# aras-p/UnityGaussianSplatting

Hardware: AMD Instinct MI355X
Metric: Msplats/s rendered (sort+view+composite+resolve), bicycle-sized synthetic 6,131,954 splats, 1200x797, Medium; ms/frame in ms_per_step (higher is better)
Workload: dtype f32; 1 GPU; bicycle-sized synthetic 6,131,954 splats, 1200x797, Medium; sort_mode=visible_in_flight, frames_in_flight=2, frames_in_flight_impl=library, splats=6131954, views=1, views_per_rank=1, blend=exact, sort_nth_frame=1, tile_pairs_P=4376060, tile=32x16, visible_splats=1563698, parallelism=single GPU, rccl_ranks=0

## Files before the change

unitygaussiansplatting_amd/csrc/gs_device_math.h:

```cpp
#pragma once
#include <stdint.h>

#if defined(__HIPCC__)
#include <hip/hip_runtime.h>
#include <hip/hip_fp16.h>
#define GS_HD __host__ __device__ __forceinline__
#else
#include <cmath>
#include <cstring>
#define GS_HD inline
#endif

#ifndef GS_CULL_EXTENT
#define GS_CULL_EXTENT 2.8285f
#endif

namespace gsm {

struct AssetView {
    const uint8_t* pos;
    const uint8_t* other;
    const uint8_t* color;
    const uint8_t* sh;
    const uint8_t* chunk;
// ... 678 lines not shown
    const float lambda2 = fmaxf(mid - radius, 0.1f);
    float dvx = cov01, dvy = lambda1 - cov00;
    const float invLen = 1.0f / sqrtf(dot2f(dvx, dvy, dvx, dvy));
    dvx *= invLen; dvy *= invLen;
    dvy = -dvy;
    const float s1 = fminf(sqrtf(2.0f * lambda1), 4096.0f), s2 = fminf(sqrtf(2.0f * lambda2), 4096.0f);
    view.axis1[0] = s1 * dvx; view.axis1[1] = s1 * dvy;
    view.axis2[0] = s2 * dvy; view.axis2[1] = s2 * (-dvx);

    const float al = fminf(col.w * P.opacityScale, 65000.0f);
    view.color[1] = f32tof16(al);
}

template <class SHSource>
GS_HD void CalcViewColor(const AssetView& a, const FrameConsts& P, uint32_t idx, ViewPartial& vp, SHSource& shsrc) {
    ViewData& view = vp.view;
    const V4 col = vp.col;
    const V3 shMin = vp.shMin, shMax = vp.shMax;
    const bool shLerp = vp.shLerp;
    const float wx = vp.wx, wy = vp.wy, wz = vp.wz;
    const float dwx = P.camx - wx, dwy = P.camy - wy, dwz = P.camz - wz;
    float ox = mrow3(P.w2o, 0, dwx, dwy, dwz), oy = mrow3(P.w2o, 1, dwx, dwy, dwz), oz = mrow3(P.w2o, 2, dwx, dwy, dwz);
    const float invN = 1.0f / sqrtf(dot3f(ox, oy, oz, ox, oy, oz));
    ox *= invN; oy *= invN; oz *= invN;
    const float dx = -ox, dy = -oy, dz = -oz;

    const bool onlySH = P.shOnly != 0;
    F2 rg = onlySH ? F2{ 0.5f, 0.5f } : F2{ col.x, col.y };
    float b = onlySH ? 0.5f : col.z;
    if (P.shOrder >= 1) {
        uint32_t shIndex = idx;
        if (a.shFmt > 3) shIndex = LoadUShort(a.other, vp.otherEnd - 2);
        shsrc.begin(a.sh + (uint64_t)shIndex * shStrideOf(a.shFmt), a.shFmt);
        const F2 minRG = { shMin.x, shMin.y }, dRG = F2{ shMax.x, shMax.y } - minRG;
        const float minB = shMin.z, dB = shMax.z - shMin.z;
        auto SHK = [&](int k) -> RGB {
            RGB s = shsrc.load_rgb(k);
            if (shLerp) { s.rg = fma2(s.rg, dRG, minRG); s.b = fmaf(s.b, dB, minB); }
            return s;
        };
        auto MUL = [](float w, const RGB& s) -> RGB { return { F2{ w, w } * s.rg, w * s.b }; };
        auto FMA = [](float w, const RGB& s, const RGB& acc) -> RGB { return { fma2(F2{ w, w }, s.rg, acc.rg), fmaf(w, s.b, acc.b) }; };
        {
            const RGB s1v = SHK(1), s2v = SHK(2), s3v = SHK(3);
            RGB t = MUL(dy, RGB{ -s1v.rg, -s1v.b });
            t = FMA(dz, s2v, t);
            t = FMA(dx, RGB{ -s3v.rg, -s3v.b }, t);
            rg = fma2(F2{ GS_SH_C1, GS_SH_C1 }, t.rg, rg); b = fmaf(GS_SH_C1, t.b, b);
        }
        if (P.shOrder >= 2) {
            const float xx = dx * dx, yy = dy * dy, zz = dz * dz;
            const float xy = dx * dy, yz = dy * dz, xz = dx * dz;
            {
                const float b4 = 1.0925484f * xy, b5 = -1.0925484f * yz, b6 = 0.3153916f * (fmaf(2.0f, zz, -xx) - yy),
                            b7 = -1.0925484f * xz, b8 = 0.5462742f * (xx - yy);
                RGB acc = MUL(b4, SHK(4));
                acc = FMA(b5, SHK(5), acc);
                acc = FMA(b6, SHK(6), acc);
                acc = FMA(b7, SHK(7), acc);
                acc = FMA(b8, SHK(8), acc);
                rg += acc.rg; b += acc.b;
            }
            if (P.shOrder >= 3) {
                const float b9 = (-0.5900436f * dy) * fmaf(3.0f, xx, -yy);
                const float b10 = (2.8906114f * xy) * dz;
                const float b11 = (-0.4570458f * dy) * (fmaf(4.0f, zz, -xx) - yy);
                const float b12 = (0.3731763f * dz) * (fmaf(2.0f, zz, -3.0f * xx) - 3.0f * yy);
                const float b13 = (-0.4570458f * dx) * (fmaf(4.0f, zz, -xx) - yy);
                const float b14 = (1.4453057f * dz) * (xx - yy);
                const float b15 = (-0.5900436f * dx) * fmaf(-3.0f, yy, xx);
                RGB acc = MUL(b9, SHK(9));
                acc = FMA(b10, SHK(10), acc);
                acc = FMA(b11, SHK(11), acc);
                acc = FMA(b12, SHK(12), acc);
                acc = FMA(b13, SHK(13), acc);
                acc = FMA(b14, SHK(14), acc);
                acc = FMA(b15, SHK(15), acc);
                rg += acc.rg; b += acc.b;
            }
        }
    }
    float r = rg.x, g = rg.y;
    r = fmaxf(r, 0.0f); g = fmaxf(g, 0.0f); b = fmaxf(b, 0.0f);
    view.color[0] = (f32tof16(r) << 16) | f32tof16(g);
    view.color[1] = (f32tof16(b) << 16) | (view.color[1] & 0xffffu);
}

template <class SHSource>
GS_HD ViewData CalcViewDataT(const AssetView& a, const FrameConsts& P, const EditView& E, uint32_t idx, SHSource& shsrc) {
    ViewPartial vp;
    CalcViewGeom(a, P, E, idx, vp);
    if (vp.front) CalcViewColor(a, P, idx, vp, shsrc);
    return vp.view;
}

GS_HD ViewData CalcViewData(const AssetView& a, const FrameConsts& P, const EditView& E, uint32_t idx) {
    SHFromBlob src;
    return CalcViewDataT(a, P, E, idx, src);
}

GS_HD void PixRange(float c, float e, float size, int& lo, int& hi) {
    float flo = ceilf((c - e) - 0.5f), fhi = floorf((c + e) - 0.5f);
    flo = fmaxf(flo, 0.0f); fhi = fminf(fhi, size - 1.0f);
    if (!(flo <= fhi)) { lo = 1; hi = 0; return; }
    lo = (int)flo; hi = (int)fhi;
}

constexpr uint32_t kAlphaThresholdBits = 0x3B808081u;
constexpr uint32_t kAlphaWindow = 16u;
constexpr uint32_t kAlphaWindowLo = kAlphaThresholdBits - kAlphaWindow / 2u;
GS_HD float Exp2Det(float y) {
    const float n = rintf(y);
    const float f = y - n;
    float p = 1.525273380405984e-05f;
    p = fmaf(p, f, 1.5403530393381608e-04f);
    p = fmaf(p, f, 1.3333558146428443e-03f);
    p = fmaf(p, f, 9.618129107628477e-03f);
    p = fmaf(p, f, 5.550410866482158e-02f);
    p = fmaf(p, f, 2.402265069591007e-01f);
    p = fmaf(p, f, 6.931471805599453e-01f);
    p = fmaf(p, f, 1.0f);
    return ldexpf(p, (int)n);
}
GS_HD float DecideAlpha(float alphaNative, float y, float a, bool& live) {
    const uint32_t u = f2u(alphaNative) - kAlphaWindowLo;
    if (u < kAlphaWindow) {
        const float ad = fminf(fmaxf(Exp2Det(y) * a, 0.0f), 1.0f);
        live = ad >= u2f(kAlphaThresholdBits);
        return ad;
    }
    live = (int32_t)u >= (int32_t)kAlphaWindow;
    return alphaNative;
}

GS_HD float LogDet(float x) {
    const uint32_t u = f2u(x);
    float e = (float)((int)(u >> 23) - 127);
    float m = u2f((u & 0x7fffffu) | 0x3f800000u);
    if (m > 1.41421356f) { m *= 0.5f; e += 1.0f; }
    const float t = (m - 1.0f) / (m + 1.0f);
    const float t2 = t * t;
    const float p = fmaf(t2, fmaf(t2, fmaf(t2, 1.0f / 7.0f, 0.2f), 1.0f / 3.0f), 1.0f);
    return fmaf(e, 0.69314718f, (2.0f * t) * p);
}

GS_HD bool BlockMayTouch(float bcx, float bcy, float half, float cx, float cy, float u1x, float u1y, float u2x, float u2y, float r2) {
    const float dx = bcx - cx, dy = bcy - cy;
    const float d1 = fabsf(fmaf(dy, u1y, dx * u1x)) - half * (fabsf(u1x) + fabsf(u1y));
    const float d2 = fabsf(fmaf(dy, u2y, dx * u2x)) - half * (fabsf(u2x) + fabsf(u2y));
    const float m1 = fmaxf(d1, 0.0f), m2 = fmaxf(d2, 0.0f);
    return (m1 <= 2.001f) && (m2 <= 2.001f) && (fmaf(m2, m2, m1 * m1) <= r2);
}

struct SplatFootprint {
    float cx, cy;
    int x0, x1, y0, y1;
};
GS_HD void PackPixelRect(const SplatFootprint& fp, uint32_t& rx, uint32_t& ry) {
    rx = (uint32_t)fp.x0 | ((uint32_t)fp.y0 << 16);
    ry = (uint32_t)(fp.x1 + 1) | ((uint32_t)(fp.y1 + 1) << 16);
}

GS_HD bool PrepareSplat(const ViewData& v, float W, float H, float nearClip, float farClip, SplatFootprint& fp) {
    fp.x0 = 1; fp.x1 = 0; fp.y0 = 1; fp.y1 = 0; fp.cx = 0.0f; fp.cy = 0.0f;
    const float w = v.pos[3];
    const float a = f16tof32(v.color[1]);
    const int drawable = (int)(w > 0.0f) & (int)(w >= nearClip) & (int)(w <= farClip) & (int)finite32(v.axis1[0]) & (int)finite32(v.axis1[1]) &
                         (int)finite32(v.axis2[0]) & (int)finite32(v.axis2[1]) & (int)(a >= 1.0f / 255.0f);
    if (!drawable) return false;
    const float invw = 1.0f / w;
    const float cx = fmaf(0.5f * (v.pos[0] * invw), W, 0.5f * W);
    const float cy = fmaf(-0.5f * (v.pos[1] * invw), H, 0.5f * H);
    const float a1x = v.axis1[0], a1y = v.axis1[1], a2x = v.axis2[0], a2y = v.axis2[1];
    const float d1 = dot2f(a1x, a1y, a1x, a1y), d2 = dot2f(a2x, a2y, a2x, a2y);
    const int inv1ok = (int)((f2u(d1) - 0x00200001u) <= (0x7f800000u - 0x00200001u)), inv2ok = (int)((f2u(d2) - 0x00200001u) <= (0x7f800000u - 0x00200001u));
    fp.cx = cx; fp.cy = cy;
    if (!((int)finite32(cx) & (int)finite32(cy) & inv1ok & inv2ok)) return false;
    const float exr = 2.0f * (fabsf(a1x) + fabsf(a2x)), eyr = 2.0f * (fabsf(a1y) + fabsf(a2y));
    const float slack = 0.01f;
    int x0, x1, y0, y1;
    PixRange(fp.cx, exr + slack, W, x0, x1);
    PixRange(fp.cy, eyr + slack, H, y0, y1);
    if (x0 > x1 || y0 > y1) return false;
    const float r2 = fmaf(LogDet(255.0f * a), 1.0001f, 1.0e-3f);
    const float rr = sqrtf(fmaxf(r2, 0.0f));
    const float exe = rr * sqrtf(dot2f(a1x, a2x, a1x, a2x)), eye = rr * sqrtf(dot2f(a1y, a2y, a1y, a2y));
    PixRange(fp.cx, fminf(exr, exe) + slack, W, x0, x1);
    PixRange(fp.cy, fminf(eyr, eye) + slack, H, y0, y1);
    if (x0 > x1 || y0 > y1) return true;
    fp.x0 = x0; fp.x1 = x1; fp.y0 = y0; fp.y1 = y1;
    return true;
}

}
```

unitygaussiansplatting_amd/csrc/gs_raster.hip:

```cpp
#include "gs_common.h"
#include <cstdlib>

namespace gs {

namespace {

struct RasterConsts {
    float W, H, nearClip, farClip;
    uint32_t tilesX, tilesY, width, height;
};

constexpr unsigned long long BFLAG_AGG = 1ull << 62, BFLAG_INCL = 2ull << 62, BVAL_MASK = (1ull << 62) - 1ull;
constexpr uint32_t BIN_SPIN_LIMIT = 1u << 24;

__device__ __forceinline__ float rl(float x, int b) { return __int_as_float(__builtin_amdgcn_readlane(__float_as_int(x), b)); }

__device__ __forceinline__ uint32_t wave_incl_scan_u32(uint32_t v) {
#define GS_DPP(x, ctrl, rowmask) (uint32_t)__builtin_amdgcn_update_dpp(0, (int)(x), ctrl, rowmask, 0xf, false)
    v += GS_DPP(v, 0x111, 0xf);
    v += GS_DPP(v, 0x112, 0xf);
    v += GS_DPP(v, 0x114, 0xf);
    v += GS_DPP(v, 0x118, 0xf);
    v += GS_DPP(v, 0x142, 0xa);
    v += GS_DPP(v, 0x143, 0xc);
// ... 571 lines not shown
            const uint32_t o = slot - s_off[e];
            const uint32_t twh = s_twh[e], tx0 = s_tx[e];
            uint32_t ty, tx;
            slot_to_xy(o, max(twh & 0xffffu, 1u), ty, tx);
            tiles[k] = __umul24((tx0 >> 16) + ty, tilesX) + (tx0 & 0xffffu) + tx;
            sids[k] = s_sid[e];
            live[k] = slot < s1;
        }
        if (live[SPT - 1]) {
            static_assert(SPT == 4, "four slots per thread");
            *(uint4*)(pairKeys + s0 + tid * SPT) = make_uint4(tiles[0], tiles[1], tiles[2], tiles[3]);
            *(uint4*)(pairVals + s0 + tid * SPT) = make_uint4(sids[0], sids[1], sids[2], sids[3]);
        } else {
#pragma unroll
            for (int k = 0; k < SPT; ++k) if (live[k]) { pairKeys[s0 + tid * SPT + k] = tiles[k]; pairVals[s0 + tid * SPT + k] = sids[k]; }
        }
#pragma unroll
        for (int k = 0; k < SPT; ++k) {
            if (live[k]) {
                if (TILECNT) atomicAdd(&s_tile[tiles[k]], 1u);
                else atomicAdd(&s_hist[tiles[k] & digitMask], 1u);
            }
            if (!TILECNT && PASSES >= 2) hist_add_aggregated(s_hist + 256, (tiles[k] >> digitBits) & digitMask, live[k]);
            if (!TILECNT && PASSES >= 3) hist_add_aggregated(s_hist + 512, (tiles[k] >> (2u * digitBits)) & digitMask, live[k]);
        }
    }
    __syncthreads();
    if (TILECNT) {
        for (uint32_t t = tid; t < kBinTileCounters; t += kEmitThreads) {
            const uint32_t c = s_tile[t];
            if (c) {
                atomicAdd(&s_hist[t & digitMask], c);
                if (PASSES >= 2) atomicAdd(&s_hist[256 + ((t >> digitBits) & digitMask)], c);
            }
        }
        __syncthreads();
    }
    uint32_t* myHist = pairHist + (bid % histCopies) * (uint32_t)kHistStride;
    for (int j = tid; j < PASSES * 256; j += kEmitThreads) {
        const uint32_t c = s_hist[j];
        if (c) atomicAdd(&myHist[j], c);
    }
}

__global__ __launch_bounds__(256) void tile_ranges_kernel(const uint32_t* __restrict__ pairKeys, const uint32_t* nPtr,
                                                          uint32_t* __restrict__ tileStart, uint32_t* __restrict__ tileEnd, uint32_t numTiles) {
    GS_CHAIN_PRIORITY();
    const uint32_t n = *nPtr;
    const uint32_t octs = (n + 7u) >> 3;
    for (uint32_t q = blockIdx.x * 256u + threadIdx.x; q < octs; q += gridDim.x * 256u) {
        const uint32_t j0 = q << 3;
        const uint4 ka = ((const uint4*)pairKeys)[2u * q], kb = ((const uint4*)pairKeys)[2u * q + 1u];
        const uint32_t k[10] = { j0 ? pairKeys[j0 - 1u] : 0xffffffffu, ka.x, ka.y, ka.z, ka.w, kb.x, kb.y, kb.z, kb.w,
                                 (j0 + 8u < n) ? pairKeys[j0 + 8u] : 0xffffffffu };
#pragma unroll
        for (int c = 0; c < 8; ++c) {
            const uint32_t j = j0 + (uint32_t)c;
            if (j >= n) break;
            const uint32_t t = k[c + 1];
            if (t >= numTiles) continue;
            if (j == 0 || k[c] != t) tileStart[t] = j;
            if (j == n - 1 || k[c + 2] != t) tileEnd[t] = j + 1;
        }
    }
}

__device__ __forceinline__ float mix_mul_lo(uint32_t h, float x) {
    float d;
    asm("v_fma_mix_f32 %0, %1, %2, 0 op_sel_hi:[1,0,0]" : "=v"(d) : "v"(h), "v"(x));
    return d;
}
__device__ __forceinline__ float mix_mul_hi(uint32_t h, float x) {
    float d;
    asm("v_fma_mix_f32 %0, %1, %2, 0 op_sel:[1,0,0] op_sel_hi:[1,0,0]" : "=v"(d) : "v"(h), "v"(x));
    return d;
}
__device__ __forceinline__ float mix_mul_lo_sat_after_trans(uint32_t h, float x) {
    float d;
    asm("s_nop 0\n\tv_fma_mix_f32 %0, %1, %2, 0 op_sel_hi:[1,0,0] clamp" : "=v"(d) : "v"(h), "v"(x));
    return d;
}
__device__ __forceinline__ float mix_one_minus_hi(uint32_t h) {
    float d;
    asm("v_fma_mix_f32 %0, %1, -1.0, 1.0 op_sel:[1,0,0] op_sel_hi:[1,0,0]" : "=v"(d) : "v"(h));
    return d;
}
__device__ __forceinline__ void mix_blend4(uint32_t& rg, uint32_t& ba, float pr, float pg, float pb, float pa, float t) {
    asm("v_fma_mixlo_f16 %0, %2, %6, %0 op_sel_hi:[0,0,1]\n\t"
        "v_fma_mixlo_f16 %1, %4, %6, %1 op_sel_hi:[0,0,1]\n\t"
        "v_fma_mixhi_f16 %0, %3, %6, %0 op_sel:[0,0,1] op_sel_hi:[0,0,1]\n\t"
        "v_fma_mixhi_f16 %1, %5, %6, %1 op_sel:[0,0,1] op_sel_hi:[0,0,1]"
        : "+v"(rg), "+v"(ba) : "v"(pr), "v"(pg), "v"(pb), "v"(pa), "v"(t));
}

__device__ __forceinline__ float half_lo(uint32_t u) { return (float)__builtin_bit_cast(_Float16, (unsigned short)(u & 0xffffu)); }
__device__ __forceinline__ float half_hi(uint32_t u) { return (float)__builtin_bit_cast(_Float16, (unsigned short)(u >> 16)); }
template <int MODE> struct PixelAcc;
template <> struct PixelAcc<0> {
    uint32_t rg, ba;
    __device__ __forceinline__ void load(uint2 d) { rg = d.x; ba = d.y; }
    __device__ __forceinline__ void blend(uint32_t c0, uint32_t c1, float alpha) {
        const float t = mix_one_minus_hi(ba);
        mix_blend4(rg, ba, mix_mul_hi(c0, alpha), mix_mul_lo(c0, alpha), mix_mul_hi(c1, alpha), alpha, t);
    }
    __device__ __forceinline__ void blend_src(float pr, float pg, float pb, float pa) { const float t = mix_one_minus_hi(ba); mix_blend4(rg, ba, pr, pg, pb, pa, t); }
    __device__ __forceinline__ bool finished() const { return (ba >> 16) == 0x3c00u; }
    __device__ __forceinline__ bool saturated() const { return false; }
    __device__ __forceinline__ uint2 pack() const { return make_uint2(rg, ba); }
};
template <> struct PixelAcc<1> {
    float r, g, b, a;
    __device__ __forceinline__ void load(uint2 d) {
        r = gsm::f16tof32(d.x); g = gsm::f16tof32(d.x >> 16); b = gsm::f16tof32(d.y); a = gsm::f16tof32(d.y >> 16);
    }
    __device__ __forceinline__ void blend(uint32_t c0, uint32_t c1, float alpha) {
        const float t = 1.0f - a;
        r = fmaf(mix_mul_hi(c0, alpha), t, r); g = fmaf(mix_mul_lo(c0, alpha), t, g); b = fmaf(mix_mul_hi(c1, alpha), t, b);
        a = fmaf(alpha, t, a);
    }
    __device__ __forceinline__ void blend_src(float pr, float pg, float pb, float pa) { const float t = 1.0f - a; r = fmaf(pr, t, r); g = fmaf(pg, t, g); b = fmaf(pb, t, b); a = fmaf(pa, t, a); }
    __device__ __forceinline__ bool finished() const { return (1.0f - a) < (1.0f / 4096.0f); }
    __device__ __forceinline__ bool saturated() const { return (1.0f - a) < (1.0f / 4096.0f); }
    __device__ __forceinline__ uint2 pack() const {
        uint2 o;
        o.x = gsm::f32tof16(r) | (gsm::f32tof16(g) << 16);
        o.y = gsm::f32tof16(b) | (gsm::f32tof16(a) << 16);
        return o;
    }
};

typedef uint32_t u4v __attribute__((ext_vector_type(4)));

#ifdef GS_BLEND_STATS
__device__ unsigned long long g_blendStats[8];
#define GS_STAT(i, v) do { if (lane == 0) atomicAdd(&g_blendStats[i], (unsigned long long)(v)); } while (0)
#else
#define GS_STAT(i, v) do { } while (0)
#endif
#ifdef GS_BLEND_TL
__device__ unsigned long long g_blendTl[8192 * 8];
#endif
template <int MODE, bool DEPTH, int TWL, int THL>
__global__ __launch_bounds__(64 << (TWL + THL - 6)) void blend_kernel(const uint32_t* __restrict__ pairVals, const uint32_t* __restrict__ tileStart,
                                                    const uint32_t* __restrict__ tileEnd, const uint32_t* __restrict__ tileOrder,
                                                    uint32_t* __restrict__ tileCost, const SplatRec* __restrict__ recs,
                                                    uint16_t* __restrict__ rt, RasterConsts rc, int dstIsZero,
                                                    const float* __restrict__ recW, const float* __restrict__ sceneDepth,
                                                    const BinControl* __restrict__ binCtl, const uint32_t* __restrict__ pairSortError,
                                                    FrameReport* __restrict__ report) {
    constexpr int TW = 1 << TWL, TH = 1 << THL;
    constexpr int NWX = TW / 8, NW = NWX * (TH / 8);
    constexpr int NT = 64 * NW;
    constexpr uint32_t SLOTS = 2048u * 256u / (uint32_t)NT;
    __shared__ float4 s_a[NT];
    __shared__ uint4 s_b[NT];
    __shared__ float4 s_e[NT];
    __shared__ int s_done;
    __shared__ uint32_t s_cost;
    uint32_t survWalked = 0;

    const int tid = threadIdx.x, lane = tid & 63, w = tid >> 6;
#ifdef GS_BLEND_TL
    const unsigned long long tl0 = wall_clock64();
#endif
    if (blockIdx.x == 0 && tid == 0) write_report(binCtl, pairSortError, report, (uint32_t)TWL | ((uint32_t)THL << 8));
    const uint32_t tile = tileOrder[blockIdx.x];
#ifndef GS_BLEND_NOPRIO
    if (blockIdx.x < SLOTS / 8u) __builtin_amdgcn_s_setprio(3);
    else if (blockIdx.x < 3u * SLOTS / 8u) __builtin_amdgcn_s_setprio(2);
    else if (blockIdx.x < 6u * SLOTS / 8u) __builtin_amdgcn_s_setprio(1);
#endif
    const uint32_t tx = tile % rc.tilesX, ty = tile / rc.tilesX;
    const uint32_t start = tileStart[tile], end = tileEnd[tile];
    const int qx0 = (int)tx * TW + (w % NWX) * 8, qy0 = (int)ty * TH + (w / NWX) * 8;
    const int px = qx0 + (lane & 7), py = qy0 + (lane >> 3);
    const bool inside = px < (int)rc.width && py < (int)rc.height;
    uint2* dst = (uint2*)(rt + ((size_t)py * rc.width + (size_t)px) * 4);
    if (start >= end) {
        if (threadIdx.x == 0) tileCost[tile] = 0;
#ifdef GS_BLEND_TL
        if (threadIdx.x == 0 && blockIdx.x < 8192u) { unsigned long long* q = g_blendTl + blockIdx.x * 8u; q[0] = tl0; q[1] = wall_clock64(); q[2] = 0; q[3] = 0; q[4] = 0; q[5] = tile; q[6] = 0; }
#endif
        if (dstIsZero && inside) *dst = make_uint2(0u, 0u);
        return;
    }
    uint32_t batchesWalked = 0;

    const float fx = (float)px + 0.5f, fy = (float)py + 0.5f;
    const gsm::F2 fxy = { fx, fy };
    const float qminx = (float)qx0 + 0.5f, qmaxx = (float)qx0 + 7.5f, qminy = (float)qy0 + 0.5f, qmaxy = (float)qy0 + 7.5f;

    PixelAcc<MODE> acc;
    float sceneZ = 0.0f;
    if (DEPTH) sceneZ = inside ? sceneDepth[(size_t)py * rc.width + (size_t)px] : 0.0f;
    acc.load((inside && !dstIsZero) ? *dst : make_uint2(0u, 0u));
    if (tid == 0) s_done = 0;
    if (tid == 0) s_cost = 0u;
    bool waveDone = false;

    const uint32_t lastPair = end - 1u;
    float4 r0, r1;
    float rw = 0.0f;
    {
        const uint32_t s0 = pairVals[min(start + (uint32_t)tid, lastPair)];
        const float4* rp = (const float4*)(recs + s0);
        r0 = rp[0]; r1 = rp[1];
        if (DEPTH) rw = recW[s0];
    }
    uint32_t sidxNext = pairVals[min(start + (uint32_t)NT + (uint32_t)tid, lastPair)];
    for (uint32_t bs = start; bs < end; bs += (uint32_t)NT) {
        __syncthreads();
        if (s_done == NW) break;
        ++batchesWalked;
        GS_STAT(0, 1);
        const uint32_t cnt = min((uint32_t)NT, end - bs);
        if ((uint32_t)tid < cnt) {
            const float inv1 = 1.0f / gsm::dot2f(r0.z, r0.w, r0.z, r0.w);
            const float inv2 = 1.0f / gsm::dot2f(r1.x, r1.y, r1.x, r1.y);
            const float ca = gsm::f16tof32(gsm::f2u(r1.w));
            const float exr = 2.0f * (fabsf(r0.z) + fabsf(r1.x)), eyr = 2.0f * (fabsf(r0.w) + fabsf(r1.y));
            const float r2 = fmaf(gsm::LogDet(255.0f * ca), 1.0001f, 1.0e-3f);
            const float rr = sqrtf(fmaxf(r2, 0.0f));
            const float exe = rr * sqrtf(gsm::dot2f(r0.z, r1.x, r0.z, r1.x)), eye = rr * sqrtf(gsm::dot2f(r0.w, r1.y, r0.w, r1.y));
            s_a[tid] = make_float4(r0.x, r0.y, r0.z * inv1, r1.x * inv2);
            s_b[tid] = make_uint4(gsm::f2u(r0.w * inv1), gsm::f2u(r1.y * inv2), gsm::f2u(r1.z), gsm::f2u(r1.w));
            s_e[tid] = make_float4(fminf(exr, exe) + 0.02f, fminf(eyr, eye) + 0.02f, r2, rw);
        }
        {
            const float4* rp = (const float4*)(recs + sidxNext);
            r0 = rp[0]; r1 = rp[1];
            if (DEPTH) rw = recW[sidxNext];
            sidxNext = pairVals[min(bs + 2u * (uint32_t)NT + (uint32_t)tid, lastPair)];
        }
        __syncthreads();
        if (!waveDone) {
            for (uint32_t c = 0; c < cnt; c += 64u) {
                const uint32_t j = c + lane;
                bool hit = false;
                GS_STAT(1, 1);
                if (j < cnt) {
                    const float4 ra = s_a[j];
                    const float4 re = s_e[j];
                    hit = (ra.x + re.x >= qminx) && (ra.x - re.x <= qmaxx) && (ra.y + re.y >= qminy) && (ra.y - re.y <= qmaxy);
#ifdef GS_BLEND_STATS
                    { const unsigned long long bb = __ballot(hit); if (__ffsll((long long)__ballot(true)) - 1 == lane) atomicAdd(&g_blendStats[2], (unsigned long long)__popcll(bb)); }
#endif
                    const uint4 rb = s_b[j];
                    hit = hit && gsm::BlockMayTouch((float)qx0 + 4.0f, (float)qy0 + 4.0f, 3.5f, ra.x, ra.y, ra.z, gsm::u2f(rb.x), ra.w, gsm::u2f(rb.y), re.z);
                }
                unsigned long long mask = __ballot(hit);
                survWalked += (uint32_t)__popcll(mask);
                auto fragment = [&](const float4 A4, const u4v B4, const uint32_t rec) {
                    const gsm::F2 d = fxy - gsm::F2{ A4.x, A4.y };
                    const gsm::F2 q = gsm::fma2(gsm::F2{ d.y, d.y }, gsm::F2{ gsm::u2f(B4.x), gsm::u2f(B4.y) }, gsm::F2{ d.x, d.x } * gsm::F2{ A4.z, A4.w });
                    const float q1 = q.x, q2 = q.y;
                    const float power = -fmaf(q2, q2, q1 * q1);
                    const float y2 = power * 1.44269504088896340736f;
                    float alpha = mix_mul_lo_sat_after_trans(B4.w, __builtin_amdgcn_exp2f(y2));
                    const int inQuad = (int)(fmaxf(fabsf(q1), fabsf(q2)) <= 2.0f);
                    bool live;
                    if (MODE == 0) {
                        const bool geHi = alpha >= gsm::u2f(gsm::kAlphaWindowLo + gsm::kAlphaWindow);
                        const bool geLo = alpha >= gsm::u2f(gsm::kAlphaWindowLo);
                        live = (inQuad & (int)geHi) != 0;
                        const bool nearT = (inQuad & (int)geLo & (int)!geHi) != 0;
                        if (__builtin_expect(__any(nearT), 0)) {
                            if (nearT) alpha = gsm::DecideAlpha(alpha, y2, half_lo(B4.w), live);
                        }
                    } else {
                        live = (inQuad & (int)(alpha >= 1.0f / 255.0f)) != 0;
                    }
                    if (DEPTH) live = live && (s_e[rec].w <= sceneZ);
                    if (MODE == 1) live = live && !acc.saturated();
#ifdef GS_BLEND_STATS
                    { const unsigned long long lv = __ballot(live); GS_STAT(4, __popcll(lv)); }
#endif
                    if (live) acc.blend(B4.z, B4.w, alpha);
                };
#ifdef GS_BLEND_PREFETCH
                if (mask) {
                    int b0 = __ffsll((long long)mask) - 1;
                    mask &= ~(1ull << b0);
                    float4 A0 = s_a[c + b0];
                    u4v B0 = *(const u4v*)&s_b[c + b0];
                    for (;;) {
                        const bool more1 = mask != 0;
                        const int b1 = more1 ? __ffsll((long long)mask) - 1 : b0;
                        mask &= ~(1ull << b1);
                        const float4 A1 = s_a[c + b1];
                        u4v B1 = *(const u4v*)&s_b[c + b1];
                        asm volatile("" : "+v"(B0));
                        fragment(A0, B0, c + (uint32_t)b0);
                        if (!more1) break;
                        const bool more0 = mask != 0;
                        b0 = more0 ? __ffsll((long long)mask) - 1 : b1;
                        mask &= ~(1ull << b0);
                        A0 = s_a[c + b0];
                        B0 = *(const u4v*)&s_b[c + b0];
                        asm volatile("" : "+v"(B1));
                        fragment(A1, B1, c + (uint32_t)b1);
                        if (!more0) break;
                    }
                }
#else
                while (mask) {
                    const int b = __ffsll((long long)mask) - 1;
                    mask &= ~(1ull << b);
                    const float4 A4 = s_a[c + b];
                    u4v B4 = *(const u4v*)&s_b[c + b];
                    asm volatile("" : "+v"(B4));
                    fragment(A4, B4, c + (uint32_t)b);
                }
#endif
                if (__all(!inside || acc.finished())) {
                    waveDone = true;
                    if (lane == 0) atomicAdd(&s_done, 1);
                    break;
                }
            }
        }
    }
    if (inside) *dst = acc.pack();
    if (lane == 0) atomicMax(&s_cost, survWalked);
    GS_STAT(3, survWalked);
    if (w == 0) GS_STAT(5, 1);
    __syncthreads();
    if (threadIdx.x == 0) tileCost[tile] = min(254u, (s_cost + batchesWalked * (uint32_t)(NT / 8)) / 4u);
#ifdef GS_BLEND_TL
    if (threadIdx.x == 0 && blockIdx.x < 8192u) {
        unsigned long long* q = g_blendTl + blockIdx.x * 8u;
        uint32_t hwid; asm volatile("s_getreg_b32 %0, hwreg(HW_REG_HW_ID)" : "=s"(hwid));
        uint32_t xcc; asm volatile("s_getreg_b32 %0, hwreg(HW_REG_XCC_ID)" : "=s"(xcc));
        q[0] = tl0; q[1] = wall_clock64(); q[2] = batchesWalked; q[3] = s_cost; q[4] = end - start; q[5] = tile; q[6] = hwid | ((unsigned long long)xcc << 32);
    }
#endif
}

__global__ __launch_bounds__(256) void splat_depth_kernel(gsm::AssetView a, gsm::FrameConsts P, const uint32_t* __restrict__ visMask32, float* __restrict__ recW) {
    const uint32_t idx = blockIdx.x * 256u + threadIdx.x;
    if (idx >= a.n || !((visMask32[idx >> 5] >> (idx & 31u)) & 1u)) return;
    const gsm::V3 pos = gsm::LoadSplatPosChunk(a, idx, blockIdx.x);
    const float wx = gsm::mrow(P.o2w, 0, pos.x, pos.y, pos.z), wy = gsm::mrow(P.o2w, 1, pos.x, pos.y, pos.z), wz = gsm::mrow(P.o2w, 2, pos.x, pos.y, pos.z);
    recW[idx] = gsm::mrow(P.vp, 3, wx, wy, wz);
}

template <bool CHUNKS>
__global__ __launch_bounds__(256) void box_setup_kernel(gsm::AssetView a, gsm::FrameConsts P, gsm::RayConsts ray, uint32_t count, gsm::BoxRec* __restrict__ recs,
                                                        uint2* __restrict__ rects, unsigned long long* __restrict__ visMask, uint8_t* __restrict__ waveFlags) {
    const uint32_t idx = blockIdx.x * 256u + threadIdx.x;
    bool visible = false;
    uint2 rect = make_uint2(0u, 0u);
    if (idx < count) {
        float c[3], B[9], r, g, b, al;
        if (!CHUNKS) {
            const gsm::V3 pos = gsm::LoadSplatPos(a, idx);
            gsm::V4 q; gsm::V3 sc; float opacity;
            gsm::LoadSplatRotScaleOpacity(a, idx, q, sc, opacity);
            const float sx = sc.x * P.splatScale, sy = sc.y * P.splatScale, sz = sc.z * P.splatScale;
            for (int k = 0; k < 3; ++k) c[k] = gsm::mrow(P.o2w, k, pos.x, pos.y, pos.z);
            const float x = q.x, y = q.y, z = q.z, w = q.w;
            const float m1[9] = { fmaf(-2.0f, fmaf(z, z, y * y), 1.0f) * sx, (2.0f * fmaf(-w, z, x * y)) * sy, (2.0f * fmaf(w, y, x * z)) * sz,
                                  (2.0f * fmaf(w, z, x * y)) * sx, fmaf(-2.0f, fmaf(z, z, x * x), 1.0f) * sy, (2.0f * fmaf(-w, x, y * z)) * sz,
                                  (2.0f * fmaf(-w, y, x * z)) * sx, (2.0f * fmaf(w, x, y * z)) * sy, fmaf(-2.0f, fmaf(y, y, x * x), 1.0f) * sz };
            for (int i = 0; i < 3; ++i)
                for (int j = 0; j < 3; ++j) B[i * 3 + j] = gsm::dot3f(P.o2w[i * 4], P.o2w[i * 4 + 1], P.o2w[i * 4 + 2], m1[j], m1[3 + j], m1[6 + j]) * 2.0f;
            const gsm::V3 col = gsm::LoadSplatBaseColor(a, idx);
            r = gsm::sat(col.x); g = gsm::sat(col.y); b = gsm::sat(col.z);
            al = gsm::sat(opacity * P.opacityScale);
        } else {
            const uint8_t* ck = a.chunk + (uint64_t)idx * 64;
            float mid[3], half[3];
            for (int k = 0; k < 3; ++k) { const float mn = gsm::u2f(gsm::ld32a(ck, 16 + 8 * k)), mx = gsm::u2f(gsm::ld32a(ck, 20 + 8 * k)); mid[k] = (mn + mx) * 0.5f; half[k] = (mx - mn) * 0.5f; }
            for (int k = 0; k < 3; ++k) c[k] = gsm::mrow(P.o2w, k, mid[0], mid[1], mid[2]);
            for (int i = 0; i < 3; ++i)
                for (int j = 0; j < 3; ++j) B[i * 3 + j] = P.o2w[i * 4 + j] * half[j];
            const float t = (float)idx / (float)count;
            r = fmaf(0.5f, cosf(6.28318f * (t + 0.0f)), 0.5f); g = fmaf(0.5f, cosf(6.28318f * (t + 0.33f)), 0.5f); b = fmaf(0.5f, cosf(6.28318f * (t + 0.67f)), 0.5f);
            al = 0.1f;
        }
        gsm::BoxRec rec;
        int x0, x1, y0, y1;
        if (gsm::BuildBox(c, B, ray, P.vp, r, g, b, al, rec, x0, x1, y0, y1)) {
            visible = true;
            rect.x = (uint32_t)x0 | ((uint32_t)y0 << 16);
            rect.y = (uint32_t)(x1 + 1) | ((uint32_t)(y1 + 1) << 16);
            uint4* rp = (uint4*)(recs + idx);
            const uint32_t* w32 = (const uint32_t*)&rec;
#pragma unroll
            for (int k = 0; k < 4; ++k) rp[k] = make_uint4(w32[4 * k], w32[4 * k + 1], w32[4 * k + 2], w32[4 * k + 3]);
        }
        rects[idx] = rect;
    }
    const unsigned long long vb = __ballot(visible);
    if ((threadIdx.x & 63u) == 0u && idx < count) visMask[idx >> 6] = vb;
    if ((threadIdx.x & 63u) == 0u && idx < count) waveFlags[idx >> 6] = vb != 0ull ? 1u : 0u;
}

template <int MODE, bool DEPTH>
__global__ __launch_bounds__(256) void blend_box_kernel(const uint32_t* __restrict__ pairVals, const uint32_t* __restrict__ tileStart,
                                                        const uint32_t* __restrict__ tileEnd, const uint32_t* __restrict__ tileOrder,
                                                        uint32_t* __restrict__ tileCost, const gsm::BoxRec* __restrict__ recs, uint16_t* __restrict__ rt,
                                                        RasterConsts rc, gsm::RayConsts ray, int dstIsZero, const float* __restrict__ sceneDepth) {
    __shared__ uint4 s_rec[64 * 4];
    const int tid = threadIdx.x;
    const uint32_t tile = tileOrder[blockIdx.x];
    const uint32_t tx = tile % rc.tilesX, ty = tile / rc.tilesX;
    const uint32_t start = tileStart[tile], end = tileEnd[tile];
    const int px = (int)tx * 16 + (tid & 15), py = (int)ty * 16 + (tid >> 4);
    const bool inside = px < (int)rc.width && py < (int)rc.height;
    uint2* dst = (uint2*)(rt + ((size_t)py * rc.width + (size_t)px) * 4);
    if (start >= end) {
        if (tid == 0) tileCost[tile] = 0;
        if (dstIsZero && inside) *dst = make_uint2(0u, 0u);
        return;
    }
    PixelAcc<MODE> acc;
    acc.load((inside && !dstIsZero) ? *dst : make_uint2(0u, 0u));
    float sceneZ = 0.0f;
    if (DEPTH) sceneZ = inside ? sceneDepth[(size_t)py * rc.width + (size_t)px] : 0.0f;
    float d[3];
    gsm::PixelRay(ray, px, py, d);
    uint32_t walked = 0;
    for (uint32_t bs = start; bs < end; bs += 64u) {
        __syncthreads();
        const uint32_t cnt = min(64u, end - bs);
        {
            const uint32_t rix = (uint32_t)tid >> 2;
            if (rix < cnt) s_rec[tid] = ((const uint4*)(recs + pairVals[bs + rix]))[tid & 3];
        }
        __syncthreads();
        ++walked;
        for (uint32_t j = 0; j < cnt; ++j) {
            const float* R = (const float*)&s_rec[j * 4];
            float ld[3];
#pragma unroll
            for (int k = 0; k < 3; ++k) ld[k] = fmaf(R[k * 3 + 2], d[2], fmaf(R[k * 3 + 1], d[1], R[k * 3] * d[0]));
            const float al = R[15];
            const float t = gsm::BoxFaceDepth(R + 9, ld, al < 0.0f);
            bool live = inside && t > 0.0f && t >= rc.nearClip && t <= rc.farClip;
            if (DEPTH) live = live && (t <= sceneZ);
            if (MODE == 1) live = live && !acc.saturated();
            const float a = fabsf(al);
            if (live) acc.blend_src(R[12] * a, R[13] * a, R[14] * a, a);
        }
    }
    if (inside) *dst = acc.pack();
    if (tid == 0) tileCost[tile] = walked * 8u;
}

__global__ __launch_bounds__(256) void debug_points_kernel(gsm::AssetView a, gsm::FrameConsts P, float halfSize, uint32_t width, uint32_t height,
                                                           const float* __restrict__ sceneDepth, unsigned long long* __restrict__ zbuf) {
    const uint32_t idx = blockIdx.x * 256u + threadIdx.x;
    if (idx >= a.n) return;
    const gsm::V3 pos = gsm::LoadSplatPos(a, idx);
    const float wx = gsm::mrow(P.o2w, 0, pos.x, pos.y, pos.z), wy = gsm::mrow(P.o2w, 1, pos.x, pos.y, pos.z), wz = gsm::mrow(P.o2w, 2, pos.x, pos.y, pos.z);
    const float cxc = gsm::mrow(P.vp, 0, wx, wy, wz), cyc = gsm::mrow(P.vp, 1, wx, wy, wz), w = gsm::mrow(P.vp, 3, wx, wy, wz);
    if (!(w >= P.nearClip && w <= P.farClip)) return;
    const float invw = 1.0f / w;
    const float cx = fmaf(0.5f * (cxc * invw), P.screenW, 0.5f * P.screenW);
    const float cy = fmaf(-0.5f * (cyc * invw), P.screenH, 0.5f * P.screenH);
    if (!(gsm::finite32(cx) && gsm::finite32(cy))) return;
    const float x0f = fmaxf(ceilf((cx - halfSize) - 0.5f), 0.0f), x1f = fminf(ceilf((cx + halfSize) - 0.5f) - 1.0f, (float)width - 1.0f);
    const float y0f = fmaxf(ceilf((cy - halfSize) - 0.5f), 0.0f), y1f = fminf(ceilf((cy + halfSize) - 0.5f) - 1.0f, (float)height - 1.0f);
    if (!(x0f <= x1f && y0f <= y1f)) return;
    const unsigned long long key = ((unsigned long long)gsm::f2u(w) << 32) | (unsigned long long)(0xffffffffu - idx);
    for (int y = (int)y0f; y <= (int)y1f; ++y)
// ... 446 lines not shown
```

Baseline: 15790 Msplats/s.

## Split blend wave into half-wave 8x4 rects with per-half splat culling

```diff
diff --git a/unitygaussiansplatting_amd/csrc/gs_device_math.h b/unitygaussiansplatting_amd/csrc/gs_device_math.h
--- a/unitygaussiansplatting_amd/csrc/gs_device_math.h
+++ b/unitygaussiansplatting_amd/csrc/gs_device_math.h
@@ -854,6 +854,23 @@
     return (m1 <= 2.001f) && (m2 <= 2.001f) && (fmaf(m2, m2, m1 * m1) <= r2);
 }
 
+GS_HD bool BlockMayTouchRect(float X2, float Y2, float HX2, float HY2, float cx, float cy, float ex, float ey, float u1x, float u1y, float u2x,
+                             float u2y, float r2) {
+    const float dx = fmaf(cx, 2.0f, -X2), dy = fmaf(cy, 2.0f, -Y2);
+    const bool box = (fabsf(dx) <= fmaf(ex, 2.0f, HX2)) && (fabsf(dy) <= fmaf(ey, 2.0f, HY2));
+    const float d1 = fabsf(fmaf(dy, u1y, dx * u1x)) - fmaf(HX2, fabsf(u1x), HY2 * fabsf(u1y));
+    const float d2 = fabsf(fmaf(dy, u2y, dx * u2x)) - fmaf(HX2, fabsf(u2x), HY2 * fabsf(u2y));
+    const float m1 = fmaxf(d1, 0.0f), m2 = fmaxf(d2, 0.0f);
+    return box && (m1 <= 2.0f * 2.001f) && (m2 <= 2.0f * 2.001f) && (fmaf(m2, m2, m1 * m1) <= 4.0f * r2);
+}
+
+GS_HD void MaskRect(uint32_t m, int x0, int y0, int& X2, int& Y2, int& HX2, int& HY2) {
+    const uint32_t cols = (m | (m >> 8) | (m >> 16) | (m >> 24)) & 0xffu;
+    const int c0 = __builtin_ctz(cols), c1 = 31 - __builtin_clz(cols), r0 = __builtin_ctz(m) >> 3, r1 = (31 - __builtin_clz(m)) >> 3;
+    X2 = 2 * x0 + 1 + c0 + c1; HX2 = c1 - c0;
+    Y2 = 2 * y0 + 1 + r0 + r1; HY2 = r1 - r0;
+}
+
 struct SplatFootprint {
     float cx, cy;
     int x0, x1, y0, y1;
diff --git a/unitygaussiansplatting_amd/csrc/gs_raster.hip b/unitygaussiansplatting_amd/csrc/gs_raster.hip
--- a/unitygaussiansplatting_amd/csrc/gs_raster.hip
+++ b/unitygaussiansplatting_amd/csrc/gs_raster.hip
@@ -747,9 +747,9 @@
     constexpr int NWX = TW / 8, NW = NWX * (TH / 8);
     constexpr int NT = 64 * NW;
     constexpr uint32_t SLOTS = 2048u * 256u / (uint32_t)NT;
-    __shared__ float4 s_a[NT];
-    __shared__ uint4 s_b[NT];
-    __shared__ float4 s_e[NT];
+    __shared__ float4 s_a[NT + 1];
+    __shared__ uint4 s_b[NT + 1];
+    __shared__ float4 s_e[NT + 1];
     __shared__ int s_done;
     __shared__ uint32_t s_cost;
     uint32_t survWalked = 0;
@@ -783,7 +783,6 @@
 
     const float fx = (float)px + 0.5f, fy = (float)py + 0.5f;
     const gsm::F2 fxy = { fx, fy };
-    const float qminx = (float)qx0 + 0.5f, qmaxx = (float)qx0 + 7.5f, qminy = (float)qy0 + 0.5f, qmaxy = (float)qy0 + 7.5f;
 
     PixelAcc<MODE> acc;
     float sceneZ = 0.0f;
@@ -791,7 +790,11 @@
     acc.load((inside && !dstIsZero) ? *dst : make_uint2(0u, 0u));
     if (tid == 0) s_done = 0;
     if (tid == 0) s_cost = 0u;
+    if (tid == 0) { s_a[NT] = make_float4(0.0f, 0.0f, 0.0f, 0.0f); s_b[NT] = make_uint4(0u, 0u, 0u, 0u); s_e[NT] = make_float4(0.0f, 0.0f, 0.0f, 0.0f); }
     bool waveDone = false;
+    const int wq = __builtin_amdgcn_readfirstlane(w);
+    const int sqx0 = (int)tx * TW + (wq % NWX) * 8, sqy0 = (int)ty * TH + (wq / NWX) * 8;
+    const uint32_t halfShift = lane < 32 ? 0u : 16u;
 
     const uint32_t lastPair = end - 1u;
     float4 r0, r1;
@@ -831,21 +834,33 @@
         if (!waveDone) {
             for (uint32_t c = 0; c < cnt; c += 64u) {
                 const uint32_t j = c + lane;
-                bool hit = false;
                 GS_STAT(1, 1);
+                const unsigned long long um = __ballot(inside && !acc.finished());
+                const uint32_t uT = (uint32_t)um, uB = (uint32_t)(um >> 32);
+                int tX2 = 0, tY2 = 0, tHX2 = 0, tHY2 = 0, bX2 = 0, bY2 = 0, bHX2 = 0, bHY2 = 0;
+                if (uT) gsm::MaskRect(uT, sqx0, sqy0, tX2, tY2, tHX2, tHY2);
+                if (uB) gsm::MaskRect(uB, sqx0, sqy0 + 4, bX2, bY2, bHX2, bHY2);
+                bool hitT = false, hitB = false;
                 if (j < cnt) {
                     const float4 ra = s_a[j];
                     const float4 re = s_e[j];
-                    hit = (ra.x + re.x >= qminx) && (ra.x - re.x <= qmaxx) && (ra.y + re.y >= qminy) && (ra.y - re.y <= qmaxy);
+                    const uint4 rb = s_b[j];
+                    hitT = gsm::BlockMayTouchRect((float)tX2, (float)tY2, (float)tHX2, (float)tHY2, ra.x, ra.y, re.x, re.y, ra.z, gsm::u2f(rb.x), ra.w, gsm::u2f(rb.y), re.z);
+                    hitB = gsm::BlockMayTouchRect((float)bX2, (float)bY2, (float)bHX2, (float)bHY2, ra.x, ra.y, re.x, re.y, ra.z, gsm::u2f(rb.x), ra.w, gsm::u2f(rb.y), re.z);
 #ifdef GS_BLEND_STATS
-                    { const unsigned long long bb = __ballot(hit); if (__ffsll((long long)__ballot(true)) - 1 == lane) atomicAdd(&g_blendStats[2], (unsigned long long)__popcll(bb)); }
+                    const float qminx = (float)qx0 + 0.5f, qmaxx = (float)qx0 + 7.5f, qminy = (float)qy0 + 0.5f, qmaxy = (float)qy0 + 7.5f;
+                    const bool box = (ra.x + re.x >= qminx) && (ra.x - re.x <= qmaxx) && (ra.y + re.y >= qminy) && (ra.y - re.y <= qmaxy);
+                    const bool quad = box && gsm::BlockMayTouch((float)qx0 + 4.0f, (float)qy0 + 4.0f, 3.5f, ra.x, ra.y, ra.z, gsm::u2f(rb.x), ra.w, gsm::u2f(rb.y), re.z);
+                    const unsigned long long bb = __ballot(box), qq = __ballot(quad);
+                    if (__ffsll((long long)__ballot(true)) - 1 == lane) { atomicAdd(&g_blendStats[2], (unsigned long long)__popcll(bb)); atomicAdd(&g_blendStats[6], (unsigned long long)__popcll(qq)); }
 #endif
-                    const uint4 rb = s_b[j];
-                    hit = hit && gsm::BlockMayTouch((float)qx0 + 4.0f, (float)qy0 + 4.0f, 3.5f, ra.x, ra.y, ra.z, gsm::u2f(rb.x), ra.w, gsm::u2f(rb.y), re.z);
                 }
-                unsigned long long mask = __ballot(hit);
-                survWalked += (uint32_t)__popcll(mask);
-                auto fragment = [&](const float4 A4, const u4v B4, const uint32_t rec) {
+                unsigned long long maskT = __ballot(hitT), maskB = __ballot(hitB);
+                if (!uT) maskT = 0ull;
+                if (!uB) maskB = 0ull;
+                survWalked += (uint32_t)max(__popcll(maskT), __popcll(maskB));
+                GS_STAT(7, __popcll(maskT) + __popcll(maskB));
+                auto fragment = [&](const float4 A4, const u4v B4, const uint32_t off) {
                     const gsm::F2 d = fxy - gsm::F2{ A4.x, A4.y };
                     const gsm::F2 q = gsm::fma2(gsm::F2{ d.y, d.y }, gsm::F2{ gsm::u2f(B4.x), gsm::u2f(B4.y) }, gsm::F2{ d.x, d.x } * gsm::F2{ A4.z, A4.w });
                     const float q1 = q.x, q2 = q.y;
@@ -865,48 +880,24 @@
                     } else {
                         live = (inQuad & (int)(alpha >= 1.0f / 255.0f)) != 0;
                     }
-                    if (DEPTH) live = live && (s_e[rec].w <= sceneZ);
+                    if (DEPTH) live = live && (((const float4*)((const char*)s_e + off))->w <= sceneZ);
                     if (MODE == 1) live = live && !acc.saturated();
 #ifdef GS_BLEND_STATS
                     { const unsigned long long lv = __ballot(live); GS_STAT(4, __popcll(lv)); }
 #endif
                     if (live) acc.blend(B4.z, B4.w, alpha);
                 };
-#ifdef GS_BLEND_PREFETCH
-                if (mask) {
-                    int b0 = __ffsll((long long)mask) - 1;
-                    mask &= ~(1ull << b0);
-                    float4 A0 = s_a[c + b0];
-                    u4v B0 = *(const u4v*)&s_b[c + b0];
-                    for (;;) {
-                        const bool more1 = mask != 0;
-                        const int b1 = more1 ? __ffsll((long long)mask) - 1 : b0;
-                        mask &= ~(1ull << b1);
-                        const float4 A1 = s_a[c + b1];
-                        u4v B1 = *(const u4v*)&s_b[c + b1];
-                        asm volatile("" : "+v"(B0));
-                        fragment(A0, B0, c + (uint32_t)b0);
-                        if (!more1) break;
-                        const bool more0 = mask != 0;
-                        b0 = more0 ? __ffsll((long long)mask) - 1 : b1;
-                        mask &= ~(1ull << b0);
-                        A0 = s_a[c + b0];
-                        B0 = *(const u4v*)&s_b[c + b0];
-                        asm volatile("" : "+v"(B1));
-                        fragment(A1, B1, c + (uint32_t)b1);
-                        if (!more0) break;
-                    }
+                while (maskT | maskB) {
+                    const int bT = __ffsll((long long)maskT) - 1, bB = __ffsll((long long)maskB) - 1;
+                    maskT &= ~(1ull << (bT & 63));
+                    maskB &= ~(1ull << (bB & 63));
+                    const uint32_t oT = (bT >= 0 ? c + (uint32_t)bT : (uint32_t)NT) * 16u, oB = (bB >= 0 ? c + (uint32_t)bB : (uint32_t)NT) * 16u;
+                    const uint32_t off = ((oT | (oB << 16)) >> halfShift) & 0xffffu;
+                    const float4 A4 = *(const float4*)((const char*)s_a + off);
+                    u4v B4 = *(const u4v*)((const char*)s_b + off);
+                    asm volatile("" : "+v"(B4));
+                    fragment(A4, B4, off);
                 }
-#else
-                while (mask) {
-                    const int b = __ffsll((long long)mask) - 1;
-                    mask &= ~(1ull << b);
-                    const float4 A4 = s_a[c + b];
-                    u4v B4 = *(const u4v*)&s_b[c + b];
-                    asm volatile("" : "+v"(B4));
-                    fragment(A4, B4, c + (uint32_t)b);
-                }
-#endif
                 if (__all(!inside || acc.finished())) {
                     waveDone = true;
                     if (lane == 0) atomicAdd(&s_done, 1);
```

Result: no change. 15700 Msplats/s, median of 2 (-0.6%).
